# WHU-USI3DV/LaneMapping

Measured on AMD Instinct MI355X. Metric: BEV tiles/sec end-to-end (LAS points -> polylines), higher is better.
Workload: dtype f32; 1 GPU; on-GPU LAS->BEV raster (4,194,304 points/tile resident in HBM) + configs/Proj_polyline_fpn_vit_vertex_2.py, batch=16 per GPU, seeded random weights; lines_per_tile=45, streams=2, hip_graphs=True, points=resident, stream_check=not run (--full runs it), gather_check=n/a (1 rank), raster_check=not run (--full runs it), dist_ranks=1, rccl_ranks=1

## Files before the change

### include/lanemap_hip.h

```cpp
#ifndef LANEMAP_HIP_H
#define LANEMAP_HIP_H
#include <stdint.h>
#ifdef __cplusplus
extern "C" {
#endif

enum { LM_OK = 0, LM_ERR_ARG = 1, LM_ERR_HIP = 2, LM_ERR_NO_DEVICE = 3 };
enum { LM_ACT_NONE = 0, LM_ACT_RELU = 1, LM_ACT_GELU = 2 };

int lm_abi_version(void);
const char* lm_last_error(void);
int lm_device_count(void);

int lm_conv2d_nhwc_mfma_f32(void* stream, const float* x, int ldx, const float* wp, int CoutP,
                            const float* scale, const float* shift, const float* res, int ldr, int res_rows,
                            float* y, int ldy, int B, int H, int W, int Cin, int Cout, int KH, int KW,
                            int stride, int pad_h, int pad_w, int dil, int act);
int lm_conv2d_nhwc_mfma_resup_f32(void* stream, const float* x, int ldx, const float* wp, int CoutP, const float* scale,
                                  const float* shift, const float* res_coarse, int ldr, int Hr, int Wr, float* y, int ldy,
                                  int B, int H, int W, int Cin, int Cout, int KH, int KW, int stride, int pad_h, int pad_w,
                                  int dil, int act);

int lm_winograd44_supported(int H, int W, int Cin, int dil);
int lm_winograd44_gn_chunks(int H, int W, int dil);
// ... 4 lines not shown
                              int Cin, int Cout, int dil, int act, double* gn_partial);
int lm_conv3x3_winograd44_twin_f32(void* stream, const float* x, int ldx, const float* wu, int CoutP, const float* scale,
                                   const float* shift, const float* res, int ldr, float* y, int ldy, int B, int H, int W,
                                   int Cin, int Cout, int dil, int act, void* workspace, long workspace_bytes);
int lm_wino44_split_fragments(void* stream, const float* frag, float* out, long n_quads);
int lm_conv3x3_winograd44_split_f32(void* stream, const float* x, int ldx, const float* wu_split, int CoutP, const float* scale,
                                    const float* shift, const float* res, int ldr, float* y, int ldy, int B, int H, int W,
                                    int Cin, int Cout, int dil, int act, double* gn_partial, float post);
int lm_conv3x3_winograd44_split_twin_f32(void* stream, const float* x, int ldx, const float* wu, int CoutP, const float* scale,
                                         const float* shift, const float* res, int ldr, float* y, int ldy, int B, int H, int W,
                                         int Cin, int Cout, int dil, int act, void* workspace, long workspace_bytes, float post);

int lm_conv2d_nhwc_mfma_f32_gnstats(void* stream, const float* x, int ldx, const float* wp, int CoutP, const float* shift,
                                    float* y, int ldy, double* gn_partial, int B, int H, int W, int Cin, int Cout,
                                    int KH, int KW, int stride, int pad_h, int pad_w, int dil);
int lm_gn_finalize(void* stream, const double* partial, float* stats, int B, int HW, int C, int nchunk, float eps);
int lm_gn_finalize_split(void* stream, const double* partial, float* stats, int B, int HW, int C, int nchunk, float eps, int split);

int lm_stem_conv7x7_bn_relu(void* stream, const float* x_chw, const float* w_k64, const float* scale,
                            const float* shift, float* y_nhwc, int B, int H, int W);
int lm_stem_conv7x7_bn_relu_u8(void* stream, const unsigned char* x_hwc3, const float* w_k64, const float* scale,
                               const float* shift, float* y_nhwc, int B, int H, int W);
int lm_maxpool3x3s2_nhwc(void* stream, const float* x, float* y, int B, int H, int W, int C);
int lm_conv2d_nhwc_small(void* stream, const float* x, int ldx, const float* w_tc16, const float* scale,
                         const float* shift, float* y, int ldy, int B, int H, int W, int Cin, int Cout,
                         int KH, int KW, int stride, int pad_h, int pad_w, int pre_relu, int act);

int lm_gn_stats(void* stream, const float* x, double* workspace, float* stats, int B, int HW, int C, float eps);
long lm_gn_stats_workspace_bytes(int B, int HW, int C);
int lm_gn_relu_upsample(void* stream, const float* x, const float* stats, const float* gamma, const float* beta,
                        float* y, int B, int Hi, int Wi, int Ho, int Wo, int C, int accumulate);
int lm_gn_relu_upsample_sum(void* stream, int n, const float* const* x, const float* const* stats, const int* Hi, const int* Wi,
                            const int* ldx , const float* gamma, const float* beta,
                            float* y, int B, int Ho, int Wo, int C);
int lm_gn_relu_upsample_sum_conv1x1(void* stream, int n, const float* const* x, const float* const* stats, const int* Hi, const int* Wi,
                                    const int* ldx, const float* gamma, const float* beta, float* y, int B, int Ho, int Wo, int C,
                                    const float* w_c16, const float* bias, int cout, float* y1, int ldy1);
int lm_upsample_bilinear_nhwc(void* stream, const float* x, int ldx, const float* add, int lda, float* y, int ldy,
                              int B, int Hi, int Wi, int Ho, int Wo, int C);
int lm_upsample_bilinear_to_chw(void* stream, const float* x, int ldx, float* y_chw, int B, int Hi, int Wi,
                                int Ho, int Wo, int C);
int lm_layernorm_rows(void* stream, const float* x, const float* gamma, const float* beta, float* y,
                      long rows, int D, float eps);
int lm_unpatchify(void* stream, const float* tokens, float* y_nhwc, int B, int G, int P, int C);
int lm_token_mix_mfma_f32(void* stream, const float* x, const float* wt, int ldw, const float* bias, const float* res, float* y,
                          int B, int M, int K, int N, int act);

int lm_attention_f32(void* stream, const float* qkv, float* out, int B, int N, int heads, int dim_head, float scale);
int lm_attention_masked_f32(void* stream, const float* qkv, float* out, const int* valid, int B, int N, int heads, int dim_head, float scale);

int lm_head_tokens(void* stream, const float* seg, const float* row_nhwc16, float* tok, float seg_bias,
                   int B, int P, int Hr, int Wr, int prop_width, int half_buff);
int lm_head_tokens_window(void* stream, const float* row_nhwc16, float* tok, int B, int P, int Hr, int Wr, int prop_width, int half_buff);
int lm_head_stage2(void* stream, const float* hid, int ldh, int D, const float* w2, const float* b2,
                   float* ext2, float* cls2, float* off2, long M);
int lm_head_proposal_conf(void* stream, const float* tok, const float* wt, const float* bias, float* conf,
                          int BP, int L);

int lm_decode_proposals(void* stream, const float* pconf, const float* ext2, const float* cls2, const float* off2,
                        float* prop_conf, float* v_ext, float* cls_conf, int* cls_idx, double* cls_offset,
                        int B, int P, int R, float exist_thre, int prop_width, int half_buff);
int lm_decode_orient(void* stream, const float* x_nhwc, int ldx, int C, unsigned char* y, long pixels);
int lm_decode_semantic(void* stream, const float* logit_chw3, unsigned char* sem, float* biseg, float* rows,
                       int B, int H, int W, float thre, int raw_mode);
long lm_endp_topk_workspace_bytes(int B);
int lm_endp_topk(void* stream, const float* endp_logit, void* workspace, int* out_idx, float* out_score,
                 int* out_status, int B, int H, int W, int clip, int K);

int lm_pack_segments(void* stream, int n, const void* const* src, const long* bytes, const long* dst_offsets, void* dst);


// ... 90 lines not shown
```

### lanemapping_amd/_lib.py

```python
import ctypes as C
import os

_HERE = os.path.dirname(os.path.abspath(__file__))
LIB_PATH = os.environ.get('LANEMAP_HIP_LIB') or os.path.join(_HERE, 'liblanemap_hip.so')

c_f32p = C.POINTER(C.c_float)
vp, i32, i64, f32 = C.c_void_p, C.c_int, C.c_long, C.c_float


class LmRasterParams(C.Structure):
    _fields_ = [('quat', C.c_float * 4), ('trans', C.c_float * 3), ('bev_img_offset', C.c_float * 2),
                ('img_reso', C.c_float * 2), ('local_min_ele', C.c_float), ('ele_reso', C.c_float),
                ('inten_lo', C.c_float), ('inten_hi', C.c_float)]


class LmLasHeader(C.Structure):
    _fields_ = [('version_major', C.c_int), ('version_minor', C.c_int), ('point_format', C.c_int), ('record_len', C.c_int),
                ('n_points', C.c_long), ('offset_to_points', C.c_long), ('scale', C.c_double * 3), ('offset', C.c_double * 3),
                ('min_xyz', C.c_double * 3), ('max_xyz', C.c_double * 3)]


SIGNATURES = {
    'lm_abi_version': (i32, []),
    'lm_last_error': (C.c_char_p, []),
    'lm_device_count': (i32, []),
    'lm_conv2d_nhwc_mfma_f32': (i32, [vp, vp, i32, vp, i32, vp, vp, vp, i32, i32, vp, i32,
                                      i32, i32, i32, i32, i32, i32, i32, i32, i32, i32, i32, i32]),
    'lm_conv2d_nhwc_mfma_resup_f32': (i32, [vp, vp, i32, vp, i32, vp, vp, vp, i32, i32, i32, vp, i32,
                                            i32, i32, i32, i32, i32, i32, i32, i32, i32, i32, i32, i32]),
    'lm_winograd44_supported': (i32, [i32, i32, i32, i32]),
    'lm_winograd44_gn_chunks': (i32, [i32, i32, i32]),
    'lm_winograd44_tiles': (i64, [i32, i32, i32, i32]),
    'lm_winograd44_twin_workspace_bytes': (i64, [i32, i32, i32, i32, i32, i32]),
    'lm_conv3x3_winograd44_f32': (i32, [vp, vp, i32, vp, i32, vp, vp, vp, i32, vp, i32, i32, i32, i32, i32, i32, i32, i32, vp]),
    'lm_conv3x3_winograd44_twin_f32': (i32, [vp, vp, i32, vp, i32, vp, vp, vp, i32, vp, i32, i32, i32, i32, i32, i32, i32, i32, vp, i64]),
    'lm_wino44_split_fragments': (i32, [vp, vp, vp, i64]),
    'lm_conv3x3_winograd44_split_f32': (i32, [vp, vp, i32, vp, i32, vp, vp, vp, i32, vp, i32, i32, i32, i32, i32, i32, i32, i32, vp, f32]),
    'lm_conv3x3_winograd44_split_twin_f32': (i32, [vp, vp, i32, vp, i32, vp, vp, vp, i32, vp, i32, i32, i32, i32, i32, i32, i32, i32, vp, i64, f32]),
    'lm_conv2d_nhwc_mfma_f32_gnstats': (i32, [vp, vp, i32, vp, i32, vp, vp, i32, vp] + [i32] * 11),
    'lm_gn_finalize': (i32, [vp, vp, vp, i32, i32, i32, i32, f32]),
    'lm_gn_finalize_split': (i32, [vp, vp, vp, i32, i32, i32, i32, f32, i32]),
    'lm_stem_conv7x7_bn_relu': (i32, [vp, vp, vp, vp, vp, vp, i32, i32, i32]),
    'lm_stem_conv7x7_bn_relu_u8': (i32, [vp, vp, vp, vp, vp, vp, i32, i32, i32]),
    'lm_maxpool3x3s2_nhwc': (i32, [vp, vp, vp, i32, i32, i32, i32]),
    'lm_conv2d_nhwc_small': (i32, [vp, vp, i32, vp, vp, vp, vp, i32, i32, i32, i32, i32, i32, i32, i32, i32, i32, i32, i32, i32]),
    'lm_gn_stats': (i32, [vp, vp, vp, vp, i32, i32, i32, f32]),
    'lm_gn_stats_workspace_bytes': (i64, [i32, i32, i32]),
    'lm_gn_relu_upsample': (i32, [vp, vp, vp, vp, vp, vp, i32, i32, i32, i32, i32, i32, i32]),
    'lm_gn_relu_upsample_sum': (i32, [vp, i32, vp, vp, vp, vp, vp, vp, vp, vp, i32, i32, i32, i32]),
    'lm_gn_relu_upsample_sum_conv1x1': (i32, [vp, i32, vp, vp, vp, vp, vp, vp, vp, vp, i32, i32, i32, i32, vp, vp, i32, vp, i32]),
    'lm_upsample_bilinear_nhwc': (i32, [vp, vp, i32, vp, i32, vp, i32, i32, i32, i32, i32, i32, i32]),
    'lm_upsample_bilinear_to_chw': (i32, [vp, vp, i32, vp, i32, i32, i32, i32, i32, i32]),
    'lm_layernorm_rows': (i32, [vp, vp, vp, vp, vp, i64, i32, f32]),
    'lm_token_mix_mfma_f32': (i32, [vp, vp, vp, i32, vp, vp, vp, i32, i32, i32, i32, i32]),
    'lm_unpatchify': (i32, [vp, vp, vp, i32, i32, i32, i32]),
    'lm_attention_f32': (i32, [vp, vp, vp, i32, i32, i32, i32, f32]),
    'lm_attention_masked_f32': (i32, [vp, vp, vp, vp, i32, i32, i32, i32, f32]),
    'lm_head_tokens': (i32, [vp, vp, vp, vp, f32, i32, i32, i32, i32, i32, i32]),
    'lm_head_tokens_window': (i32, [vp, vp, vp, i32, i32, i32, i32, i32, i32]),
    'lm_head_stage2': (i32, [vp, vp, i32, i32, vp, vp, vp, vp, vp, i64]),
    'lm_head_proposal_conf': (i32, [vp, vp, vp, vp, vp, i32, i32]),
    'lm_decode_proposals': (i32, [vp, vp, vp, vp, vp, vp, vp, vp, vp, vp, i32, i32, i32, f32, i32, i32]),
    'lm_decode_orient': (i32, [vp, vp, i32, i32, vp, i64]),
    'lm_decode_semantic': (i32, [vp, vp, vp, vp, vp, i32, i32, i32, f32, i32]),
    'lm_endp_topk_workspace_bytes': (i64, [i32]),
    'lm_endp_topk': (i32, [vp, vp, vp, vp, vp, vp, i32, i32, i32, i32, i32]),
    'lm_pack_segments': (i32, [vp, i32, vp, vp, vp, vp]),
    'lm_bev_raster_workspace_bytes': (i64, [i32, i64, i32, i32]),
    'lm_bev_raster_batch': (i32, [vp, vp, C.POINTER(i64), C.POINTER(LmRasterParams), i32, vp, i64, vp, vp, i32, i32]),
    'lm_tile_ingest_u8': (i32, [vp, vp, vp, i32, i32, i32, i32]),
    'lm_endp_cluster': (i32, [vp, i32, i32, i32, i32, i32, i32, i32, i32, vp, i32, vp, vp]),
    'lm_polyline_assemble': (i32, [vp, vp, vp, vp, vp, i32, i32, i32, f32, i32, vp, vp]),
    'lm_raster_polylines': (i32, [vp, i32, i32, vp]),
    'lm_line8': (i32, [vp, i32, i32, i32, i32, i32]),
    'lm_trace_lines': (i32, [vp, i32, i32, vp, vp]),
    'lm_polyline_backproject': (i32, [vp, i32, i32, i32, vp, vp, i32, i32, vp, vp, vp]),
    'lm_skeletonize_lee_2d': (i64, [vp, i32, i32]),
    'lm_merge_create': (vp, []),
    'lm_merge_destroy': (None, [vp]),
# ... 62 lines not shown
```

### lanemapping_amd/csrc/conv_direct.hip

```cpp
#include "common.h"

#include <type_traits>

typedef float f32x4 __attribute__((ext_vector_type(4)));

namespace {

constexpr int ST = 16;
constexpr int SP = 2 * ST + 5;
constexpr int SPP = 40;

template <bool U8>
__global__ __launch_bounds__(256) void stem_kernel(const void* __restrict__ xin, const float* __restrict__ w,
                                                   const float* __restrict__ scale, const float* __restrict__ shift,
                                                   float* __restrict__ y, int H, int W, int Ho, int Wo) {
    __shared__ float in[3][SP][SPP];
    const int tid = threadIdx.x;
    const int b = blockIdx.z;
    const int oy0 = blockIdx.y * ST, ox0 = blockIdx.x * ST;
    const int iy0 = oy0 * 2 - 3, ix0 = ox0 * 2 - 3;
    for (int i = tid; i < 3 * SP * SP; i += 256) {
        const int c = i / (SP * SP), r = (i / SP) % SP, q = i % SP;
        const int iy = iy0 + r, ix = ix0 + q;
        float v = 0.f;
// ... 135 lines not shown
            __builtin_amdgcn_sched_barrier(0);
        }
        float* const yt = y + (((long)b * Ho + oy0) * Wo + ox0) * 64;
        const unsigned lbyte = (unsigned)((4 * wave * Wo + 4 * half) * 64 + l32) << 2;
        auto store_tile = [&](auto guarded) {
#pragma unroll
            for (int mb = 0; mb < 2; ++mb)
#pragma unroll
                for (int r = 0; r < 16; ++r) {
                    const int ry = 2 * mb + (r >> 3), cx = (r & 3) + 8 * ((r >> 2) & 1);
                    char* const rowp = reinterpret_cast<char*>(yt) + (long)((ry * Wo + cx) * 64) * 4;
                    if (!decltype(guarded)::value || (oy0 + 4 * wave + ry < Ho && ox0 + cx + 4 * half < Wo)) {
#pragma unroll
                        for (int nb = 0; nb < 2; ++nb)
                            *reinterpret_cast<float*>(rowp + nb * 128 + lbyte) = fmaxf(acc[mb][nb][r] * sc[nb] + sh[nb], 0.f);
                    }
                }
        };
        if (oy0 + ST <= Ho && ox0 + ST <= Wo) store_tile(std::false_type{});
        else store_tile(std::true_type{});
    }
}

__global__ __launch_bounds__(256) void maxpool3x3s2_kernel(const float* __restrict__ x, float* __restrict__ y,
                                                           int H, int W, int C, int Ho, int Wo, long total4) {
    const long i = (long)blockIdx.x * 256 + threadIdx.x;
    if (i >= total4) return;
    const int c4 = C / 4;
    const int c = (int)(i % c4);
    long t = i / c4;
    const int ox = (int)(t % Wo);
    t /= Wo;
    const int oy = (int)(t % Ho);
    const int b = (int)(t / Ho);
    f32x4 m = {-INFINITY, -INFINITY, -INFINITY, -INFINITY};
#pragma unroll
    for (int dy = 0; dy < 3; ++dy)
#pragma unroll
        for (int dx = 0; dx < 3; ++dx) {
            const int iy = oy * 2 - 1 + dy, ix = ox * 2 - 1 + dx;
            if ((unsigned)iy < (unsigned)H && (unsigned)ix < (unsigned)W) {
                const f32x4 v = *reinterpret_cast<const f32x4*>(x + (((long)b * H + iy) * W + ix) * C + c * 4);
#pragma unroll
                for (int e = 0; e < 4; ++e) m[e] = fmaxf(m[e], v[e]);
            }
        }
// ... 47 lines not shown
            float v = acc[n];
            if (p.scale) v *= p.scale[n];
            if (p.shift) v += p.shift[n];
            if (p.act == LM_ACT_RELU) v = fmaxf(v, 0.f);
            yp[n] = v;
        }
    }
}

template <bool U8>
int launch_stem(void* stream, const void* x, const float* w_k64, const float* scale, const float* shift, float* y, int B, int H, int W, int Ho,
                int Wo) {
    static const bool valu = [] { const char* e = getenv("LM_STEM_VALU"); return e && atoi(e) != 0; }();
    const int tx = lm_cdiv(Wo, ST), ty = lm_cdiv(Ho, ST);
    if (valu) {
        hipLaunchKernelGGL(stem_kernel<U8>, dim3(tx, ty, B), dim3(256), 0, (hipStream_t)stream, x, w_k64, scale, shift, y, H, W, Ho, Wo);
    } else {
        const long ntiles = (long)tx * ty * B;
        LM_REQUIRE(ntiles < (1L << 31), "stem: too many tiles");
        const int grid = (int)(ntiles < 512 ? ntiles : 512);
        hipLaunchKernelGGL(stem_mfma_kernel<U8>, dim3(grid), dim3(256), 0, (hipStream_t)stream, x, w_k64, scale, shift, y, H, W, Ho, Wo,
                           lm_fastdiv_make((unsigned)tx), lm_fastdiv_make((unsigned)ty), (int)ntiles);
    }
    LM_LAUNCH_CHECK();
    return LM_OK;
}

template <int STRIDE>
__global__ __launch_bounds__(256) void small_conv3x3_mfma_kernel(SmallConvParams p, LmFastDiv div_tx, LmFastDiv div_ty, int ntiles) {
    constexpr int R = 15 * STRIDE + 3;
    extern __shared__ __attribute__((aligned(16))) float patch[];
    const int tid = threadIdx.x, lane = tid & 63, wave = tid >> 6;
    const int l16 = lane & 15, h = lane >> 4;
    float wr[9][4];
#pragma unroll
    for (int t = 0; t < 9; ++t)
#pragma unroll
        for (int j = 0; j < 4; ++j) wr[t][j] = p.w[(t * 16 + 4 * j + h) * 16 + l16];
    float sc = 1.f, sh = 0.f;
    const bool has_sc = p.scale != nullptr, has_sh = p.shift != nullptr;
    if (has_sc && l16 < p.Cout) sc = p.scale[l16];
    if (has_sh && l16 < p.Cout) sh = p.shift[l16];
    for (int t = blockIdx.x; t < ntiles; t += gridDim.x) {
        const unsigned trow = lm_fastdiv((unsigned)t, div_tx);
        const int b = (int)lm_fastdiv(trow, div_ty);
        const int oy0 = (int)(trow - (unsigned)b * div_ty.d) * 16, ox0 = (int)((unsigned)t - trow * div_tx.d) * 16;
// ... 190 lines not shown
    }
}

int launch_small_wide(const SmallConvParams& p, hipStream_t stream) {
    const bool s1 = p.stride == 1;
    if (p.Cin == 8) return s1 ? launch_small_mfma_wide_nb<1, 8>(p, stream) : launch_small_mfma_wide_nb<2, 8>(p, stream);
    return s1 ? launch_small_mfma_wide_nb<1, 16>(p, stream) : launch_small_mfma_wide_nb<2, 16>(p, stream);
}

}

LM_API int lm_stem_conv7x7_bn_relu(void* stream, const float* x_chw, const float* w_k64, const float* scale,
                                   const float* shift, float* y_nhwc, int B, int H, int W) {
    LM_REQUIRE(x_chw && w_k64 && scale && shift && y_nhwc, "stem: null pointer");
    const int Ho = (H + 6 - 7) / 2 + 1, Wo = (W + 6 - 7) / 2 + 1;
    return launch_stem<false>(stream, (const void*)x_chw, w_k64, scale, shift, y_nhwc, B, H, W, Ho, Wo);
}

LM_API int lm_stem_conv7x7_bn_relu_u8(void* stream, const unsigned char* x_hwc3, const float* w_k64, const float* scale,
                                      const float* shift, float* y_nhwc, int B, int H, int W) {
    LM_REQUIRE(x_hwc3 && w_k64 && scale && shift && y_nhwc, "stem_u8: null pointer");
    const int Ho = (H + 6 - 7) / 2 + 1, Wo = (W + 6 - 7) / 2 + 1;
    return launch_stem<true>(stream, (const void*)x_hwc3, w_k64, scale, shift, y_nhwc, B, H, W, Ho, Wo);
}

LM_API int lm_maxpool3x3s2_nhwc(void* stream, const float* x, float* y, int B, int H, int W, int C) {
    LM_REQUIRE(x && y && C % 4 == 0, "maxpool: bad args (C=%d)", C);
    const int Ho = (H + 2 - 3) / 2 + 1, Wo = (W + 2 - 3) / 2 + 1;
    const long total4 = (long)B * Ho * Wo * (C / 4);
    hipLaunchKernelGGL(maxpool3x3s2_kernel, dim3(lm_cdiv(total4, 256)), dim3(256), 0, (hipStream_t)stream,
                       x, y, H, W, C, Ho, Wo, total4);
    LM_LAUNCH_CHECK();
    return LM_OK;
}

LM_API int lm_conv2d_nhwc_small(void* stream, const float* x, int ldx, const float* w_tc16, const float* scale,
                                const float* shift, float* y, int ldy, int B, int H, int W, int Cin, int Cout,
                                int KH, int KW, int stride, int pad_h, int pad_w, int pre_relu, int act) {
    LM_REQUIRE(x && w_tc16 && y, "small_conv: null pointer");
    LM_REQUIRE(Cin % 4 == 0 && ldx % 4 == 0 && Cout >= 1 && (Cout <= 16 || (Cout <= 64 && Cout % 16 == 0)),
               "small_conv: Cin=%d (mult of 4) Cout=%d (<= 16, or 32 / 48 / 64)", Cin, Cout);
    SmallConvParams p;
    p.x = x; p.w = w_tc16; p.scale = scale; p.shift = shift; p.y = y;
    p.ldx = ldx; p.ldy = ldy; p.B = B; p.H = H; p.W = W; p.Cin = Cin; p.Cout = Cout;
    p.KH = KH; p.KW = KW; p.stride = stride; p.pad_h = pad_h; p.pad_w = pad_w; p.pre_relu = pre_relu; p.act = act;
    p.Ho = (H + 2 * pad_h - KH) / stride + 1;
// ... 26 lines not shown
```

### lanemapping_amd/csrc/vit.hip

```cpp
#include "common.h"

namespace {

constexpr int DH = 64;
constexpr int QC = 36;
constexpr int KLD = DH + 1;

__global__ __launch_bounds__(256) void attention_kernel(const float* __restrict__ qkv, float* __restrict__ out, int NT,
                                                        int heads, float scale, const int* __restrict__ valid) {
    extern __shared__ __attribute__((aligned(16))) float smem[];
    __shared__ int kidx[64];
    __shared__ int kcount;
    const int tid = threadIdx.x;
    const int q0 = blockIdx.x * QC, h = blockIdx.y, b = blockIdx.z;
    const int inner = heads * DH;
    const long row0 = (long)b * NT;
    const int ld = 3 * inner;
    int N = NT;
    if (valid) {
        if (tid < 64) {
            const bool v = tid < NT && valid[(long)b * NT + tid] != 0;
            const unsigned long long m = __ballot(v);
            if (v) kidx[__popcll(m & ((1ull << tid) - 1ull))] = tid;
            if (tid == 0) kcount = (int)__popcll(m);
// ... 57 lines not shown
    __syncthreads();
    const int d = lane;
    float acc[QC / 4];
#pragma unroll
    for (int r = 0; r < QC / 4; ++r) acc[r] = 0.f;
    for (int j = 0; j < N; ++j) {
        const float v = KV[j * KLD + d];
#pragma unroll
        for (int r = 0; r < QC / 4; ++r) acc[r] = fmaf(S[(wave + 4 * r) * SLD + j], v, acc[r]);
    }
#pragma unroll
    for (int r = 0; r < QC / 4; ++r) {
        const int i = q0 + wave + 4 * r;
        if (i < NT) out[(row0 + i) * inner + h * DH + d] = acc[r];
    }
}

typedef float f32x16 __attribute__((ext_vector_type(16)));
typedef float f32x4 __attribute__((ext_vector_type(4)));
constexpr int NKB = 11;
constexpr int NPAD = NKB * 32;
constexpr int KP = DH + 4;

__global__ __launch_bounds__(256) void attention_mfma_kernel(const float* __restrict__ qkv, float* __restrict__ out, int N, int heads,
                                                             float scale) {
    extern __shared__ __attribute__((aligned(16))) float smem[];
    const int tid = threadIdx.x, lane = tid & 63, wave = tid >> 6;
    const int h = blockIdx.y, b = blockIdx.z;
    const int inner = heads * DH, ld = 3 * inner;
    const long row0 = (long)b * N;
    const int col = lane & 31, half = lane >> 5;
    const int q = (blockIdx.x * 4 + wave) * 32 + col;
    for (int i = tid; i < NPAD * (DH / 4); i += 256) {
        const int n = i >> 4, c4 = (i & 15) * 4;
        f32x4 v = {0.f, 0.f, 0.f, 0.f};
        if (n < N) v = *reinterpret_cast<const f32x4*>(qkv + (row0 + n) * ld + inner + h * DH + c4);
        *reinterpret_cast<f32x4*>(smem + n * KP + c4) = v;
    }
    f32x4 qf[8];
#pragma unroll
    for (int g = 0; g < 8; ++g) {
        qf[g] = f32x4{0.f, 0.f, 0.f, 0.f};
        if (q < N) qf[g] = *reinterpret_cast<const f32x4*>(qkv + (row0 + q) * ld + h * DH + 8 * g + 4 * half);
    }
    __syncthreads();
    f32x16 s[NKB];
#pragma unroll
    for (int kb = 0; kb < NKB; ++kb) {
// ... 140 lines not shown
            }
        }
    }
    l += __shfl_xor(l, 32);
    if (q < N) {
        const float inv = 1.0f / l;
        float* orow = out + (row0 + q) * inner + h * DH;
#pragma unroll
        for (int dt = 0; dt < 2; ++dt)
#pragma unroll
            for (int r4 = 0; r4 < 4; ++r4) {
                f32x4 v = {o[dt][4 * r4] * inv, o[dt][4 * r4 + 1] * inv, o[dt][4 * r4 + 2] * inv, o[dt][4 * r4 + 3] * inv};
                *reinterpret_cast<f32x4*>(orow + dt * 32 + 8 * r4 + 4 * half) = v;
            }
    }
}

}

LM_API int lm_attention_f32(void* stream, const float* qkv, float* out, int B, int N, int heads, int dim_head, float scale) {
    LM_REQUIRE(qkv && out, "attention: null pointer");
    LM_REQUIRE(dim_head == DH, "attention: dim_head=%d must be %d", dim_head, DH);
    if (N > NPAD - 32 && N <= NPAD) {
        const size_t lds_m = (size_t)NPAD * KP * sizeof(float);
        if (int e = lm_ensure_dynamic_lds((const void*)attention_mfma_kernel, lds_m)) return e;
        hipLaunchKernelGGL(attention_mfma_kernel, dim3(lm_cdiv(lm_cdiv(N, 32), 4), heads, B), dim3(256), lds_m, (hipStream_t)stream, qkv, out,
                           N, heads, scale);
        LM_LAUNCH_CHECK();
        return LM_OK;
    }
    const size_t lds = ((size_t)N * KLD + (size_t)QC * (N + 4) + QC * DH) * sizeof(float);
    if (lds > 160 * 1024) {
        const size_t lds_f = (size_t)FKB * (KP + VP) * sizeof(float);
        if (int e = lm_ensure_dynamic_lds((const void*)attention_flash_kernel, lds_f)) return e;
        hipLaunchKernelGGL(attention_flash_kernel, dim3(lm_cdiv(lm_cdiv(N, 32), 4), heads, B), dim3(256), lds_f, (hipStream_t)stream, qkv,
                           out, N, heads, scale);
        LM_LAUNCH_CHECK();
        return LM_OK;
    }
    if (int e = lm_ensure_dynamic_lds((const void*)attention_kernel, lds)) return e;
    hipLaunchKernelGGL(attention_kernel, dim3(lm_cdiv(N, QC), heads, B), dim3(256), lds, (hipStream_t)stream, qkv, out, N, heads, scale,
                       (const int*)nullptr);
    LM_LAUNCH_CHECK();
    return LM_OK;
}

LM_API int lm_attention_masked_f32(void* stream, const float* qkv, float* out, const int* valid, int B, int N, int heads, int dim_head,
                                   float scale) {
    LM_REQUIRE(qkv && out && valid, "attention_masked: null pointer");
    LM_REQUIRE(dim_head == DH && N >= 1 && N <= 64, "attention_masked: dim_head=%d must be %d, N=%d at most 64", dim_head, DH, N);
    const size_t lds = ((size_t)N * KLD + (size_t)QC * (N + 4) + QC * DH) * sizeof(float);
    if (int e = lm_ensure_dynamic_lds((const void*)attention_kernel, lds)) return e;
    hipLaunchKernelGGL(attention_kernel, dim3(lm_cdiv(N, QC), heads, B), dim3(256), lds, (hipStream_t)stream, qkv, out, N, heads, scale, valid);
    LM_LAUNCH_CHECK();
    return LM_OK;
}
```

### lanemapping_amd/ops.py

```python
import ctypes as C
import math

import torch

from ._lib import lib, check, LmRasterParams, LanemapHipError

ACT_NONE, ACT_RELU, ACT_GELU = 0, 1, 2


def _stream():
    return C.c_void_p(torch._C._cuda_getCurrentRawStream(torch._C._cuda_getDevice()))


def _ptr(t):
    if t is None:
        return None
    if not t.is_cuda:
        raise LanemapHipError('lanemapping_amd ops need tensors on an MI355X (HIP) device; no CPU fallback exists')
    if t.device.index != torch._C._cuda_getDevice():
        raise LanemapHipError(f'tensor on cuda:{t.device.index} but the current device is cuda:{torch._C._cuda_getDevice()}: '
                              'call torch.cuda.set_device() (one process drives one GPU)')
    return C.c_void_p(t.data_ptr())


# ... 268 lines not shown
    B, cin, H, W = x.shape
    ph, pw = (pad, pad) if isinstance(pad, int) else pad
    Ho = (H + 2 * ph - kh) // stride + 1
    Wo = (W + 2 * pw - kw) // stride + 1
    if out is None:
        out = new_act(B, cout, Ho, Wo, x.device)
    out_, ldy = as_nhwc(out)
    assert out_.data_ptr() == out.data_ptr()
    check(lib().lm_conv2d_nhwc_small(_stream(), _ptr(x), ldx, _ptr(w16), _ptr(scale), _ptr(shift), _ptr(out), ldy,
                                     B, H, W, cin, cout, kh, kw, stride, ph, pw, int(pre_relu), act))
    return out


def stem(x, w_k64, scale, shift):
    x = x.contiguous()
    if x.dtype == torch.uint8:
        B, H, W, C_ = x.shape
        assert C_ == 3, 'u8 tiles are [B,H,W,3]'
    else:
        B, _, H, W = x.shape
    Ho, Wo = (H - 1) // 2 + 1, (W - 1) // 2 + 1
    out = new_act(B, 64, Ho, Wo, x.device)
    fn = lib().lm_stem_conv7x7_bn_relu_u8 if x.dtype == torch.uint8 else lib().lm_stem_conv7x7_bn_relu
    check(fn(_stream(), _ptr(x), _ptr(w_k64), _ptr(scale), _ptr(shift), _ptr(out), B, H, W))
    return out


def maxpool3x3s2(x):
    x, ld = as_nhwc(x)
    B, C_, H, W = x.shape
    assert ld == C_
    out = new_act(B, C_, (H - 1) // 2 + 1, (W - 1) // 2 + 1, x.device)
    check(lib().lm_maxpool3x3s2_nhwc(_stream(), _ptr(x), _ptr(out), B, H, W, C_))
    return out


def gn_stats(x, eps=1e-5):
    x, ld = as_nhwc(x)
    B, C_, H, W = x.shape
    assert ld == C_
    ws = torch.empty(lib().lm_gn_stats_workspace_bytes(B, H * W, C_) // 8, device=x.device, dtype=torch.float64)
    stats = torch.empty((B, C_, 2), device=x.device, dtype=torch.float32)
    check(lib().lm_gn_stats(_stream(), _ptr(x), _ptr(ws), _ptr(stats), B, H * W, C_, eps))
    return stats


# ... 401 lines not shown
```

### lanemapping_amd/pcencoder.py

```python
import os

import torch
import torch.nn as nn

from . import ops, trace
from .registry import PCENCODER
from .packing import PackedModule

_LAYERS = {'resnet18': [2, 2, 2, 2], 'resnet34': [3, 4, 6, 3]}
MERGE_BRANCH_CONVS = os.environ.get('LANEMAP_MERGE_BRANCH_CONVS', '1') != '0'
WINO_F44 = os.environ.get('LANEMAP_WINO_F44', '1') != '0'
WINO_F44_MIN_CIN = int(os.environ.get('LANEMAP_WINO_F44_MIN_CIN', '64'))
WINO_SPLIT = os.environ.get('LANEMAP_WINO_SPLIT', '0') != '0'


def _frag44(w):
    if WINO_SPLIT:
        return ops.pack_wino44_fragments_split(ops.pack_wino44(w))
    return ops.pack_wino44_fragments(ops.pack_wino44(w))


def _f44_ok(conv):
    return WINO_F44 and conv.kernel_size == (3, 3) and conv.stride == (1, 1) and conv.in_channels >= WINO_F44_MIN_CIN and conv.in_channels % 16 == 0

# ... 154 lines not shown
        s4 = ops.gn_relu_upsample_sum([(t, st)], P[gn_a + '.g'], P[gn_a + '.b'], (h, w))
        terms = [pre[0] if pre is not None and pre[0] is not None else self._conv_stats(P, p2, conv_b, c_half, gn_b),
                 pre[1] if pre is not None and pre[1] is not None else self._conv_stats(P, p3, conv_b, c_half, gn_b)]
        terms.append(self._conv_stats(P, s4, conv_b, c_half, gn_b))
        return ops.gn_relu_upsample_sum(terms, P[gn_b + '.g'], P[gn_b + '.b'], (h, w), proj=proj, keep_sum=False)

    def forward(self, x, fea_up_out=None):
        from . import torch_ops
        if self.out is None:
            return self._forward_impl(x, fea_up_out)
        if fea_up_out is None:
            B, H, W = (x.shape[0], x.shape[1], x.shape[2]) if x.dtype == torch.uint8 else (x.shape[0], x.shape[2], x.shape[3])
            fea_up_out = ops.new_act(B, 8, (H + 3) // 4, (W + 3) // 4, x.device)
        fea, bi_seg, endp = torch_ops.fpn_encoder(x, fea_up_out, torch_ops.stage_weights(self), torch_ops.stage_name(self))
        return fea, fea_up_out, bi_seg, endp

    def _forward_impl(self, x, fea_up_out=None):
        P = self.packed()
        if x.dtype == torch.uint8:
            B, H, W, _ = x.shape
        else:
            B, _, H, W = x.shape
        with trace.stage('fpn.stem'):
            c1 = ops.maxpool3x3s2(ops.stem(x, P['stem_w'], P['stem_s'], P['stem_b']))
        feats = []
        t = c1
        for lname in ('layer1', 'layer2', 'layer3'):
            with trace.stage('fpn.' + lname):
                for i, blk in enumerate(getattr(self, lname)):
                    t = self._block(t, P, f'{lname}.{i}', blk)
            feats.append(t)
        c2, c3, c4 = feats
        trace.push('fpn.topdown')
        fea = ops.conv_mfma(c4, P['out.w'], self.out.out_channels) if self.out is not None else None
        p4 = ops.conv_mfma(c4, P['toplayer.w'], 256, shift=P['toplayer.b'])
        def lateral(c, name, coarse):
            if tuple(coarse.shape[2:]) == tuple(c.shape[2:]):
                return ops.conv_mfma(c, P[name + '.w'], 256, shift=P[name + '.b'], res=coarse)
            return ops.conv_mfma(c, P[name + '.w'], 256, shift=P[name + '.b'], res_up=coarse)

        p3 = lateral(c3, 'latlayer1', p4)
        p2 = lateral(c2, 'latlayer2', p3)
        del c1, c2, c3, c4, feats, t
        p4 = self._conv3(p4, P, 'smooth1', 256)
        p3 = self._conv3(p3, P, 'smooth2', 256)
        p2 = self._conv3(p2, P, 'smooth3', 256)
        trace.pop()
# ... 41 lines not shown
```

Measured before the change: 396.8 tiles/s.

## Fuse stem conv+BN+ReLU with maxpool and stage attention K/V in chunks

Adds a persistent stem kernel that runs the 7x7 conv through MFMA and applies BN, ReLU and the 3x3 stride-2 maxpool in LDS. A carry row links vertical tiles, so the full-resolution stem activation is never written to HBM. It also rewrites the attention MFMA kernel to stage K and V in two chunks of 6 key blocks, which cuts LDS use and allows two blocks per CU. The old attention kernel is kept as a reference entry point. The risks are extra recompute across segment boundaries, more complex tiling, and higher register pressure.

```diff
diff --git a/include/lanemap_hip.h b/include/lanemap_hip.h
--- a/include/lanemap_hip.h
+++ b/include/lanemap_hip.h
@@ -50,6 +50,10 @@
 int lm_stem_conv7x7_bn_relu_u8(void* stream, const unsigned char* x_hwc3, const float* w_k64, const float* scale,
                                const float* shift, float* y_nhwc, int B, int H, int W);
 int lm_maxpool3x3s2_nhwc(void* stream, const float* x, float* y, int B, int H, int W, int C);
+int lm_stem_conv7x7_bn_relu_maxpool(void* launch_stream, const float* x_chw, const float* w_k64, const float* scale,
+                                    const float* shift, float* y_nhwc, int B, int H, int W);
+int lm_stem_conv7x7_bn_relu_maxpool_u8(void* launch_stream, const unsigned char* x_hwc3, const float* w_k64, const float* scale,
+                                       const float* shift, float* y_nhwc, int B, int H, int W);
 int lm_conv2d_nhwc_small(void* stream, const float* x, int ldx, const float* w_tc16, const float* scale,
                          const float* shift, float* y, int ldy, int B, int H, int W, int Cin, int Cout,
                          int KH, int KW, int stride, int pad_h, int pad_w, int pre_relu, int act);
@@ -75,6 +79,7 @@
                           int B, int M, int K, int N, int act);
 
 int lm_attention_f32(void* stream, const float* qkv, float* out, int B, int N, int heads, int dim_head, float scale);
+int lm_attention_f32_ref(void* launch_stream, const float* qkv, float* out, int B, int N, int heads, int dim_head, float scale);
 int lm_attention_masked_f32(void* stream, const float* qkv, float* out, const int* valid, int B, int N, int heads, int dim_head, float scale);
 
 int lm_head_tokens(void* stream, const float* seg, const float* row_nhwc16, float* tok, float seg_bias,
diff --git a/lanemapping_amd/_lib.py b/lanemapping_amd/_lib.py
--- a/lanemapping_amd/_lib.py
+++ b/lanemapping_amd/_lib.py
@@ -43,6 +43,8 @@
     'lm_stem_conv7x7_bn_relu': (i32, [vp, vp, vp, vp, vp, vp, i32, i32, i32]),
     'lm_stem_conv7x7_bn_relu_u8': (i32, [vp, vp, vp, vp, vp, vp, i32, i32, i32]),
     'lm_maxpool3x3s2_nhwc': (i32, [vp, vp, vp, i32, i32, i32, i32]),
+    'lm_stem_conv7x7_bn_relu_maxpool': (i32, [vp, vp, vp, vp, vp, vp, i32, i32, i32]),
+    'lm_stem_conv7x7_bn_relu_maxpool_u8': (i32, [vp, vp, vp, vp, vp, vp, i32, i32, i32]),
     'lm_conv2d_nhwc_small': (i32, [vp, vp, i32, vp, vp, vp, vp, i32, i32, i32, i32, i32, i32, i32, i32, i32, i32, i32, i32, i32]),
     'lm_gn_stats': (i32, [vp, vp, vp, vp, i32, i32, i32, f32]),
     'lm_gn_stats_workspace_bytes': (i64, [i32, i32, i32]),
@@ -55,6 +57,7 @@
     'lm_token_mix_mfma_f32': (i32, [vp, vp, vp, i32, vp, vp, vp, i32, i32, i32, i32, i32]),
     'lm_unpatchify': (i32, [vp, vp, vp, i32, i32, i32, i32]),
     'lm_attention_f32': (i32, [vp, vp, vp, i32, i32, i32, i32, f32]),
+    'lm_attention_f32_ref': (i32, [vp, vp, vp, i32, i32, i32, i32, f32]),
     'lm_attention_masked_f32': (i32, [vp, vp, vp, vp, i32, i32, i32, i32, f32]),
     'lm_head_tokens': (i32, [vp, vp, vp, vp, f32, i32, i32, i32, i32, i32, i32]),
     'lm_head_tokens_window': (i32, [vp, vp, vp, i32, i32, i32, i32, i32, i32]),
diff --git a/lanemapping_amd/csrc/conv_direct.hip b/lanemapping_amd/csrc/conv_direct.hip
--- a/lanemapping_amd/csrc/conv_direct.hip
+++ b/lanemapping_amd/csrc/conv_direct.hip
@@ -181,6 +181,188 @@
     }
 }
 
+constexpr int SPC = 14;
+constexpr int SPT = ST * ST * 32;
+
+struct StemPoolGeom {
+    int H, W, Ho, Wo, Hp, Wp;
+    int nstrips, nty, seglen, nseg, nunits;
+};
+
+template <bool U8>
+__global__ __launch_bounds__(256, 2) void stem_pool_mfma_kernel(const void* __restrict__ xin, const float* __restrict__ w,
+                                                                const float* __restrict__ scale, const float* __restrict__ shift,
+                                                                float* __restrict__ y, StemPoolGeom g) {
+    static_assert(SPT >= SP * SMW, "the pool tile aliases the patch");
+    extern __shared__ __attribute__((aligned(16))) float lds[];
+    float* const in = lds;
+    float* const wl = lds + SPT;
+    float* const u8lut = wl + SMJ * 2 * 64;
+    float* const carry = u8lut + 256;
+    const int H = g.H, W = g.W;
+    u8lut[threadIdx.x] = (float)threadIdx.x / 255.0f;
+    const int tid = threadIdx.x, lane = tid & 63, wave = tid >> 6;
+    const int l32 = lane & 31, half = lane >> 5;
+    for (int i = tid; i < SMJ * 2 * 64; i += 256) {
+        const int j = i >> 7, nb = (i >> 6) & 1, l = i & 63;
+        const int ky = (2 * j) / 22, idx = (2 * j) % 22 + (l >> 5);
+        wl[i] = idx == 21 ? 0.f : w[(ky * 21 + idx) * 64 + nb * 32 + (l & 31)];
+    }
+    float sc[2], sh[2];
+#pragma unroll
+    for (int nb = 0; nb < 2; ++nb) {
+        sc[nb] = scale[nb * 32 + l32];
+        sh[nb] = shift[nb * 32 + l32];
+    }
+    int abase[2];
+#pragma unroll
+    for (int mb = 0; mb < 2; ++mb) abase[mb] = (2 * (4 * wave + 2 * mb + (l32 >> 4))) * SMW + (2 * (l32 & 15)) * 3 + half;
+    constexpr int NST = (SP * SMW + 255) / 256;
+    int poff[NST], prq[NST];
+#pragma unroll
+    for (int k = 0; k < NST; ++k) {
+        const int i = tid + k * 256;
+        const int r = i / SMW, e = i - r * SMW;
+        const int q = e / 3, c = e - q * 3;
+        const bool cell = i < SP * SMW && q < SP;
+        poff[k] = U8 ? (r * W + q) * 3 + c : c * H * W + r * W + q;
+        prq[k] = cell ? (r << 16) | q : -1;
+    }
+    struct Pos { int unit, b, s, ty0, ty, end; };
+    auto enter = [&](Pos& p) {
+        if (p.unit >= g.nunits) return;
+        const int col = p.unit / g.nseg, seg = p.unit - col * g.nseg;
+        p.b = col / g.nstrips;
+        p.s = col - p.b * g.nstrips;
+        p.ty0 = seg * g.seglen;
+        p.end = min(p.ty0 + g.seglen, g.nty);
+        p.ty = p.ty0 > 0 ? p.ty0 - 1 : 0;
+    };
+    auto advance = [&](Pos& p) {
+        if (++p.ty >= p.end) {
+            p.unit += gridDim.x;
+            enter(p);
+        }
+    };
+    unsigned raw[NST], okmask = 0;
+    auto fetch = [&](const Pos& p) {
+        const int iy0 = p.ty * (2 * ST) - 3, ix0 = (p.s * SPC - 1) * 2 - 3;
+        const long base = U8 ? (((long)p.b * H + iy0) * W + ix0) * 3 : ((long)p.b * 3 * H + iy0) * W + ix0;
+        okmask = 0;
+#pragma unroll
+        for (int k = 0; k < NST; ++k) {
+            const int r = prq[k] >> 16, q = prq[k] & 0xffff;
+            const bool ok = (prq[k] >= 0) & ((unsigned)(iy0 + r) < (unsigned)H) & ((unsigned)(ix0 + q) < (unsigned)W);
+            okmask |= ok ? 1u << k : 0u;
+            const long src = ok ? base + poff[k] : 0;
+            if (U8) raw[k] = static_cast<const unsigned char*>(xin)[src];
+            else raw[k] = static_cast<const unsigned*>(xin)[src];
+        }
+    };
+    Pos cur;
+    cur.unit = blockIdx.x;
+    enter(cur);
+    if (cur.unit < g.nunits) fetch(cur);
+    while (cur.unit < g.nunits) {
+        const bool pre = cur.ty < cur.ty0;
+        const int oy0 = cur.ty * ST, ox0 = cur.s * SPC - 1;
+        __syncthreads();
+        if (cur.ty == 0)
+            for (int i = tid; i < ST * 64; i += 256) carry[i] = -INFINITY;
+#pragma unroll
+        for (int k = 0; k < NST; ++k) {
+            const int i = tid + k * 256;
+            const float val = U8 ? u8lut[raw[k] & 255u] : __uint_as_float(raw[k]);
+            if (i < SP * SMW) in[i] = (okmask >> k) & 1u ? val : 0.f;
+        }
+        __syncthreads();
+        Pos nxt = cur;
+        advance(nxt);
+        if (nxt.unit < g.nunits) fetch(nxt);
+        f32x16s acc[2][2];
+#pragma unroll
+        for (int mb = 0; mb < 2; ++mb)
+#pragma unroll
+            for (int nb = 0; nb < 2; ++nb)
+#pragma unroll
+                for (int r = 0; r < 16; ++r) acc[mb][nb][r] = 0.f;
+        if (!pre || wave == 3) {
+            float av[2][2], wv[2][2];
+            auto rd = [&](int j, float (&a)[2], float (&wq)[2]) {
+                const int koff = ((2 * j) / 22) * SMW + (2 * j) % 22;
+#pragma unroll
+                for (int mb = 0; mb < 2; ++mb) a[mb] = in[abase[mb] + koff];
+#pragma unroll
+                for (int nb = 0; nb < 2; ++nb) wq[nb] = wl[(j * 2 + nb) * 64 + lane];
+            };
+            rd(0, av[0], wv[0]);
+#pragma unroll
+            for (int j = 0; j < SMJ; ++j) {
+                if (j + 1 < SMJ) rd(j + 1, av[(j + 1) & 1], wv[(j + 1) & 1]);
+                __builtin_amdgcn_sched_barrier(0);
+#pragma unroll
+                for (int mb = 0; mb < 2; ++mb)
+#pragma unroll
+                    for (int nb = 0; nb < 2; ++nb)
+                        acc[mb][nb] = __builtin_amdgcn_mfma_f32_32x32x2f32(av[j & 1][mb], wv[j & 1][nb], acc[mb][nb], 0, 0, 0);
+                __builtin_amdgcn_sched_barrier(0);
+            }
+        }
+#pragma unroll
+        for (int mb = 0; mb < 2; ++mb)
+#pragma unroll
+            for (int r = 0; r < 16; ++r) {
+                const int ry = 4 * wave + 2 * mb + (r >> 3), cx = (r & 3) + 8 * ((r >> 2) & 1) + 4 * half;
+                const bool inside = oy0 + ry < g.Ho && (unsigned)(ox0 + cx) < (unsigned)g.Wo;
+#pragma unroll
+                for (int nb = 0; nb < 2; ++nb) acc[mb][nb][r] = inside ? fmaxf(acc[mb][nb][r] * sc[nb] + sh[nb], 0.f) : -INFINITY;
+            }
+        if (!pre) {
+#pragma unroll
+            for (int nb = 0; nb < 2; ++nb) {
+                __syncthreads();
+#pragma unroll
+                for (int mb = 0; mb < 2; ++mb)
+#pragma unroll
+                    for (int r = 0; r < 16; ++r) {
+                        const int ry = 4 * wave + 2 * mb + (r >> 3), cx = (r & 3) + 8 * ((r >> 2) & 1) + 4 * half;
+                        in[(ry * ST + cx) * 32 + l32] = acc[mb][nb][r];
+                    }
+                __syncthreads();
+                for (int i = tid; i < 8 * 7 * 8; i += 256) {
+                    const int cq = i & 7, pc = (i >> 3) % 7, pr = (i >> 3) / 7;
+                    const int py = cur.ty * 8 + pr, px = cur.s * 7 + pc;
+                    if (py >= g.Hp || px >= g.Wp) continue;
+                    f32x4 m = {-INFINITY, -INFINITY, -INFINITY, -INFINITY};
+#pragma unroll
+                    for (int dy = 0; dy < 3; ++dy) {
+                        const int ry = 2 * pr - 1 + dy;
+                        const float* const row = ry < 0 ? carry + nb * 32 + 4 * cq : in + ry * ST * 32 + 4 * cq;
+                        const int cstride = ry < 0 ? 64 : 32;
+#pragma unroll
+                        for (int dx = 0; dx < 3; ++dx) {
+                            const f32x4 v = *reinterpret_cast<const f32x4*>(row + (2 * pc + dx) * cstride);
+#pragma unroll
+                            for (int e = 0; e < 4; ++e) m[e] = fmaxf(m[e], v[e]);
+                        }
+                    }
+                    *reinterpret_cast<f32x4*>(y + (((long)cur.b * g.Hp + py) * g.Wp + px) * 64 + nb * 32 + 4 * cq) = m;
+                }
+            }
+        }
+        __syncthreads();
+        if (wave == 3) {
+#pragma unroll
+            for (int r = 8; r < 16; ++r) {
+                const int cx = (r & 3) + 8 * ((r >> 2) & 1) + 4 * half;
+#pragma unroll
+                for (int nb = 0; nb < 2; ++nb) carry[cx * 64 + nb * 32 + l32] = acc[1][nb][r];
+            }
+        }
+        cur = nxt;
+    }
+}
+
 __global__ __launch_bounds__(256) void maxpool3x3s2_kernel(const float* __restrict__ x, float* __restrict__ y,
                                                            int H, int W, int C, int Ho, int Wo, long total4) {
     const long i = (long)blockIdx.x * 256 + threadIdx.x;
@@ -274,6 +456,36 @@
         hipLaunchKernelGGL(stem_mfma_kernel<U8>, dim3(grid), dim3(256), 0, (hipStream_t)stream, x, w_k64, scale, shift, y, H, W, Ho, Wo,
                            lm_fastdiv_make((unsigned)tx), lm_fastdiv_make((unsigned)ty), (int)ntiles);
     }
+    LM_LAUNCH_CHECK();
+    return LM_OK;
+}
+
+template <bool U8>
+int launch_stem_pool(void* stream, const void* x, const float* w_k64, const float* scale, const float* shift, float* y, int B, int H, int W) {
+    StemPoolGeom g;
+    g.H = H; g.W = W;
+    g.Ho = (H + 6 - 7) / 2 + 1; g.Wo = (W + 6 - 7) / 2 + 1;
+    g.Hp = (g.Ho - 1) / 2 + 1; g.Wp = (g.Wo - 1) / 2 + 1;
+    g.nstrips = lm_cdiv(g.Wp, 7);
+    g.nty = lm_cdiv(g.Hp, 8);
+    LM_REQUIRE((long)B * g.nstrips * g.nty < (1L << 30), "stem_pool: too many tiles");
+    const int slots = 512;
+    long best = -1;
+    for (int len = 1; len <= g.nty; ++len) {
+        const int nseg = lm_cdiv(g.nty, len);
+        const long units = (long)B * g.nstrips * nseg;
+        const long cost = ((units + slots - 1) / slots) * (2 * len + (nseg > 1 ? 1 : 0));
+        if (best < 0 || cost < best) {
+            best = cost;
+            g.seglen = len;
+            g.nseg = nseg;
+        }
+    }
+    g.nunits = B * g.nstrips * g.nseg;
+    const size_t lds = (size_t)(SPT + SMJ * 2 * 64 + 256 + ST * 64) * sizeof(float);
+    if (int e = lm_ensure_dynamic_lds((const void*)stem_pool_mfma_kernel<U8>, lds)) return e;
+    const int grid = g.nunits < slots ? g.nunits : slots;
+    hipLaunchKernelGGL(stem_pool_mfma_kernel<U8>, dim3(grid), dim3(256), lds, (hipStream_t)stream, x, w_k64, scale, shift, y, g);
     LM_LAUNCH_CHECK();
     return LM_OK;
 }
@@ -510,6 +722,18 @@
     LM_REQUIRE(x_hwc3 && w_k64 && scale && shift && y_nhwc, "stem_u8: null pointer");
     const int Ho = (H + 6 - 7) / 2 + 1, Wo = (W + 6 - 7) / 2 + 1;
     return launch_stem<true>(stream, (const void*)x_hwc3, w_k64, scale, shift, y_nhwc, B, H, W, Ho, Wo);
+}
+
+LM_API int lm_stem_conv7x7_bn_relu_maxpool(void* stream, const float* x_chw, const float* w_k64, const float* scale,
+                                           const float* shift, float* y_nhwc, int B, int H, int W) {
+    LM_REQUIRE(x_chw && w_k64 && scale && shift && y_nhwc, "stem_pool: null pointer");
+    return launch_stem_pool<false>(stream, (const void*)x_chw, w_k64, scale, shift, y_nhwc, B, H, W);
+}
+
+LM_API int lm_stem_conv7x7_bn_relu_maxpool_u8(void* stream, const unsigned char* x_hwc3, const float* w_k64, const float* scale,
+                                              const float* shift, float* y_nhwc, int B, int H, int W) {
+    LM_REQUIRE(x_hwc3 && w_k64 && scale && shift && y_nhwc, "stem_pool_u8: null pointer");
+    return launch_stem_pool<true>(stream, (const void*)x_hwc3, w_k64, scale, shift, y_nhwc, B, H, W);
 }
 
 LM_API int lm_maxpool3x3s2_nhwc(void* stream, const float* x, float* y, int B, int H, int W, int C) {
diff --git a/lanemapping_amd/csrc/vit.hip b/lanemapping_amd/csrc/vit.hip
--- a/lanemapping_amd/csrc/vit.hip
+++ b/lanemapping_amd/csrc/vit.hip
@@ -103,8 +103,111 @@
 constexpr int NPAD = NKB * 32;
 constexpr int KP = DH + 4;
 
-__global__ __launch_bounds__(256) void attention_mfma_kernel(const float* __restrict__ qkv, float* __restrict__ out, int N, int heads,
-                                                             float scale) {
+constexpr int AKB = 6;
+
+__global__ __launch_bounds__(256, 2) void attention_mfma_kernel(const float* __restrict__ qkv, float* __restrict__ out, int N, int heads,
+                                                                float scale) {
+    extern __shared__ __attribute__((aligned(16))) float smem[];
+    const int tid = threadIdx.x, lane = tid & 63, wave = tid >> 6;
+    const int h = blockIdx.y, b = blockIdx.z;
+    const int inner = heads * DH, ld = 3 * inner;
+    const long row0 = (long)b * N;
+    const int col = lane & 31, half = lane >> 5;
+    const int q = (blockIdx.x * 4 + wave) * 32 + col;
+    auto stage = [&](int kb0, int nkb, int off, int rowld) {
+        for (int i = tid; i < nkb * 32 * (DH / 4); i += 256) {
+            const int n = i >> 4, c4 = (i & 15) * 4;
+            const int key = kb0 * 32 + n;
+            f32x4 v = {0.f, 0.f, 0.f, 0.f};
+            if (key < N) v = *reinterpret_cast<const f32x4*>(qkv + (row0 + key) * ld + off + h * DH + c4);
+            *reinterpret_cast<f32x4*>(smem + n * rowld + c4) = v;
+        }
+    };
+    f32x4 qf[8];
+#pragma unroll
+    for (int g = 0; g < 8; ++g) {
+        qf[g] = f32x4{0.f, 0.f, 0.f, 0.f};
+        if (q < N) qf[g] = *reinterpret_cast<const f32x4*>(qkv + (row0 + q) * ld + h * DH + 8 * g + 4 * half);
+    }
+    f32x16 s[NKB];
+#pragma unroll
+    for (int st = 0; st < 2; ++st) {
+        if (st) __syncthreads();
+        stage(st * AKB, st ? NKB - AKB : AKB, inner, KP);
+        __syncthreads();
+#pragma unroll
+        for (int kk = 0; kk < AKB; ++kk) {
+            const int kb = st * AKB + kk;
+            if (kb < NKB) {
+#pragma unroll
+                for (int r = 0; r < 16; ++r) s[kb][r] = 0.f;
+#pragma unroll
+                for (int g = 0; g < 8; ++g) {
+                    const f32x4 kf = *reinterpret_cast<const f32x4*>(smem + (kk * 32 + col) * KP + 8 * g + 4 * half);
+#pragma unroll
+                    for (int t = 0; t < 4; ++t) s[kb] = __builtin_amdgcn_mfma_f32_32x32x2f32(kf[t], qf[g][t], s[kb], 0, 0, 0);
+                }
+            }
+        }
+    }
+    float m = -INFINITY;
+#pragma unroll
+    for (int kb = 0; kb < NKB; ++kb)
+#pragma unroll
+        for (int r = 0; r < 16; ++r) {
+            const int key = kb * 32 + (r & 3) + 8 * (r >> 2) + 4 * half;
+            s[kb][r] = key < N ? s[kb][r] * scale : -INFINITY;
+            m = fmaxf(m, s[kb][r]);
+        }
+    m = fmaxf(m, __shfl_xor(m, 32));
+    float sum = 0.f;
+#pragma unroll
+    for (int kb = 0; kb < NKB; ++kb)
+#pragma unroll
+        for (int r = 0; r < 16; ++r) {
+            const float e = expf(s[kb][r] - m);
+            s[kb][r] = e;
+            sum += e;
+        }
+    sum += __shfl_xor(sum, 32);
+    f32x16 o[2];
+#pragma unroll
+    for (int dt = 0; dt < 2; ++dt)
+#pragma unroll
+        for (int r = 0; r < 16; ++r) o[dt][r] = 0.f;
+#pragma unroll
+    for (int st = 0; st < 2; ++st) {
+        __syncthreads();
+        stage(st * AKB, st ? NKB - AKB : AKB, 2 * inner, DH);
+        __syncthreads();
+#pragma unroll
+        for (int kk = 0; kk < AKB; ++kk) {
+            const int kb = st * AKB + kk;
+            if (kb < NKB) {
+#pragma unroll
+                for (int r = 0; r < 16; ++r) {
+                    const float* vrow = smem + (kk * 32 + (r & 3) + 8 * (r >> 2) + 4 * half) * DH + col;
+                    o[0] = __builtin_amdgcn_mfma_f32_32x32x2f32(vrow[0], s[kb][r], o[0], 0, 0, 0);
+                    o[1] = __builtin_amdgcn_mfma_f32_32x32x2f32(vrow[32], s[kb][r], o[1], 0, 0, 0);
+                }
+            }
+        }
+    }
+    if (q < N) {
+        const float inv = 1.0f / sum;
+        float* orow = out + (row0 + q) * inner + h * DH;
+#pragma unroll
+        for (int dt = 0; dt < 2; ++dt)
+#pragma unroll
+            for (int r4 = 0; r4 < 4; ++r4) {
+                f32x4 v = {o[dt][4 * r4] * inv, o[dt][4 * r4 + 1] * inv, o[dt][4 * r4 + 2] * inv, o[dt][4 * r4 + 3] * inv};
+                *reinterpret_cast<f32x4*>(orow + dt * 32 + 8 * r4 + 4 * half) = v;
+            }
+    }
+}
+
+__global__ __launch_bounds__(256) void attention_mfma_ref_kernel(const float* __restrict__ qkv, float* __restrict__ out, int N, int heads,
+                                                                 float scale) {
     extern __shared__ __attribute__((aligned(16))) float smem[];
     const int tid = threadIdx.x, lane = tid & 63, wave = tid >> 6;
     const int h = blockIdx.y, b = blockIdx.z;
@@ -291,7 +394,7 @@
     LM_REQUIRE(qkv && out, "attention: null pointer");
     LM_REQUIRE(dim_head == DH, "attention: dim_head=%d must be %d", dim_head, DH);
     if (N > NPAD - 32 && N <= NPAD) {
-        const size_t lds_m = (size_t)NPAD * KP * sizeof(float);
+        const size_t lds_m = (size_t)AKB * 32 * KP * sizeof(float);
         if (int e = lm_ensure_dynamic_lds((const void*)attention_mfma_kernel, lds_m)) return e;
         hipLaunchKernelGGL(attention_mfma_kernel, dim3(lm_cdiv(lm_cdiv(N, 32), 4), heads, B), dim3(256), lds_m, (hipStream_t)stream, qkv, out,
                            N, heads, scale);
@@ -310,6 +413,18 @@
     if (int e = lm_ensure_dynamic_lds((const void*)attention_kernel, lds)) return e;
     hipLaunchKernelGGL(attention_kernel, dim3(lm_cdiv(N, QC), heads, B), dim3(256), lds, (hipStream_t)stream, qkv, out, N, heads, scale,
                        (const int*)nullptr);
+    LM_LAUNCH_CHECK();
+    return LM_OK;
+}
+
+LM_API int lm_attention_f32_ref(void* stream, const float* qkv, float* out, int B, int N, int heads, int dim_head, float scale) {
+    if (!(N > NPAD - 32 && N <= NPAD)) return lm_attention_f32(stream, qkv, out, B, N, heads, dim_head, scale);
+    LM_REQUIRE(qkv && out, "attention: null pointer");
+    LM_REQUIRE(dim_head == DH, "attention: dim_head=%d must be %d", dim_head, DH);
+    const size_t lds_m = (size_t)NPAD * KP * sizeof(float);
+    if (int e = lm_ensure_dynamic_lds((const void*)attention_mfma_ref_kernel, lds_m)) return e;
+    hipLaunchKernelGGL(attention_mfma_ref_kernel, dim3(lm_cdiv(lm_cdiv(N, 32), 4), heads, B), dim3(256), lds_m, (hipStream_t)stream, qkv, out,
+                       N, heads, scale);
     LM_LAUNCH_CHECK();
     return LM_OK;
 }
diff --git a/lanemapping_amd/ops.py b/lanemapping_amd/ops.py
--- a/lanemapping_amd/ops.py
+++ b/lanemapping_amd/ops.py
@@ -314,6 +314,20 @@
     Ho, Wo = (H - 1) // 2 + 1, (W - 1) // 2 + 1
     out = new_act(B, 64, Ho, Wo, x.device)
     fn = lib().lm_stem_conv7x7_bn_relu_u8 if x.dtype == torch.uint8 else lib().lm_stem_conv7x7_bn_relu
+    check(fn(_stream(), _ptr(x), _ptr(w_k64), _ptr(scale), _ptr(shift), _ptr(out), B, H, W))
+    return out
+
+
+def stem_pool(x, w_k64, scale, shift):
+    x = x.contiguous()
+    if x.dtype == torch.uint8:
+        B, H, W, C_ = x.shape
+        assert C_ == 3, 'u8 tiles are [B,H,W,3]'
+    else:
+        B, _, H, W = x.shape
+    Ho, Wo = (H - 1) // 2 + 1, (W - 1) // 2 + 1
+    out = new_act(B, 64, (Ho - 1) // 2 + 1, (Wo - 1) // 2 + 1, x.device)
+    fn = lib().lm_stem_conv7x7_bn_relu_maxpool_u8 if x.dtype == torch.uint8 else lib().lm_stem_conv7x7_bn_relu_maxpool
     check(fn(_stream(), _ptr(x), _ptr(w_k64), _ptr(scale), _ptr(shift), _ptr(out), B, H, W))
     return out
 
diff --git a/lanemapping_amd/pcencoder.py b/lanemapping_amd/pcencoder.py
--- a/lanemapping_amd/pcencoder.py
+++ b/lanemapping_amd/pcencoder.py
@@ -200,7 +200,7 @@
         else:
             B, _, H, W = x.shape
         with trace.stage('fpn.stem'):
-            c1 = ops.maxpool3x3s2(ops.stem(x, P['stem_w'], P['stem_s'], P['stem_b']))
+            c1 = ops.stem_pool(x, P['stem_w'], P['stem_s'], P['stem_b'])
         feats = []
         t = c1
         for lname in ('layer1', 'layer2', 'layer3'):
```

Measured after the change: 398.5 tiles/s, median of 6. About the same (+0.4%).
